# mfkiwl/erlangnetwork-gnsslib-sdr

Measured on AMD Instinct MI355X. Metric: correlations/sec (1 ms coh) + x real-time, 32-SV L1CA @16.368 Msps, higher is better.
Workload: dtype int8 samples x int8 carrier LUT -> int32 accumulators (exact); NCOs: the reference's fp64 running sums, bit for bit; 1 GPU; BASELINE configs[2]: 32-SV GPS L1CA tracking, 5-tap E/P/L correlators (CORRN=2, CORRD=3), 1 ms coherent, 16.368 Msps int8 IQ, per GPU; channels_per_gpu=32, epochs_per_launch=1000, taps=5, loop=open (frequencies held per launch); see closed_loop (--full), if_broadcast=none (1 GPU)

## Files before the change

### erlangnetwork-gnsslib-sdr_amd/csrc/gnsscorr_nco.h

```cpp
#pragma once

#include <math.h>
#include <stdint.h>
#include <string.h>
#include <type_traits>

#if defined(__HIPCC__)
#define GC_HD __host__ __device__ inline
#define GC_HDM __host__ __device__
#define GC_HD_NOINLINE __host__ __device__ __attribute__((noinline))
#else
#define GC_HD static inline
#define GC_HDM
#define GC_HD_NOINLINE static
#endif
#if defined(__clang__)
#define GC_FP_STRICT _Pragma("clang fp contract(off)")
#else
#define GC_FP_STRICT
#endif

#if defined(__HIP_DEVICE_COMPILE__)
#define GC_DDIV(a, b) __ddiv_rn((a), (b))
#else
// ... 567 lines not shown
    } else if (!(reach < gc_u2d((uint64_t)(f.ex0 + GC_NB) << 52))) {
        return false;
    }
    c->exact = gc_cert_exact(x, f.s, reach);
    *pi0 = i0;
    *pilim = ilim;
    return true;
}

struct GcFillLoop {
    GC_HDM bool operator()(int *K, const GcCertCtx &c, int i0, int itop, double lim) const
    {
        int prev = 0;
        for (int i = i0 + 1; i <= GC_NB; i++) {
            K[i] = (i <= itop || i == GC_NB) ? gc_cert_lane(c, i, lim) : GC_CERT_FAR;
            if (K[i] == GC_CERT_FAIL) return false;
            if (i <= itop || i == GC_NB) {
                if (K[i] <= prev && !(K[i] == GC_CERT_FAR && (i != GC_NB || !(lim < 1.0e300)))) return false;
                prev = K[i];
            }
        }
        return true;
    }
};

#if defined(__HIPCC__)
struct GcFillLanes {
    int lane;
    __device__ bool operator()(int *K, const GcCertCtx &c, int i0, int itop, double lim) const
    {
        int Kl = GC_CERT_FAR;
        const bool mine = lane > i0 && lane <= GC_NB && (lane <= itop || lane == GC_NB);
        if (mine) Kl = gc_cert_lane(c, lane, lim);
        const int src = lane == GC_NB ? itop : lane - 1;
        const int below = __shfl(Kl, src < 0 ? 0 : src, 64);
        const bool bad = mine && (Kl == GC_CERT_FAIL || (src > i0 && Kl <= below && !(Kl == GC_CERT_FAR && (lane != GC_NB || !(lim < 1.0e300)))) || Kl <= 0);
        if (__any(bad)) return false;
#pragma unroll
        for (int i = 0; i <= GC_NB; i++) K[i] = __builtin_amdgcn_readlane(Kl, i);
        return true;
    }
};
#endif

template <class Fill>
GC_HD bool gc_cert_stretch(const GcNcoFast &f, double *px, int *pk, int n, double lim, Fill &fill)
{
    GcCertCtx c;
    int i0, ilim;
    if (!gc_cert_setup(f, *px, *pk, n, lim, &c, &i0, &ilim)) return false;
    const int klim = gc_cert_lane(c, GC_NB, lim);
    if (klim == GC_CERT_FAIL) return false;
    int K[GC_NB + 1];
    if (!fill(K, c, i0, ilim, klim == GC_CERT_FAR ? INFINITY : lim)) return false;
    double y = *px;
    int k = 0;
    if (!gc_cert_chain(f, &y, &k, c.n, i0, K, ilim, K[GC_NB])) return false;
    *px = y;
    *pk += k;
    return true;
}

template <class Fill>
GC_HD bool gc_plan_code_walk(const GcNcoFast &f, double c, int len, int nt, Fill &fill, double *cend)
{
    GC_FP_STRICT
    const double ci = f.s, dlen = (double)len;
    if (f.ex0 == GC_NO_TABLE || !(ci > 0.0)) return false;
    int j = 0;
    while (j < nt) {
        if (c >= dlen) c = c - dlen;
        while (j < nt && c < dlen && (c == 0.0 || gc_expo(c) < f.ex0)) {
            c = c + ci;
            j += 1;
        }
        if (j >= nt) break;
        if (c >= dlen) continue;
        if (!(c > 0.0) || !gc_cert_stretch(f, &c, &j, nt, dlen, fill)) return false;
    }
    *cend = c;
    return true;
}

GC_HD bool gc_one_binade_walk(double x, double s, int n, double *xn, double *dout = nullptr, bool *tie_out = nullptr)
{
    GC_FP_STRICT
    const uint64_t ux = gc_d2u(x), us = gc_d2u(s);
    if (tie_out) *tie_out = false;
    const int ex = gc_expo(x), es = gc_expo(s);
    if (ex == 0 || ex == 0x7FF || es == 0 || es == 0x7FF || (ux >> 63) != (us >> 63)) return false;
    const int et = es + 1075 - ex;
    if (et >= 1023 + 51) return false;
    double b = 0.0;
    if (et >= 1023 - 1) {
        const double t = gc_u2d((us & 0x800FFFFFFFFFFFFFull) | ((uint64_t)et << 52));
        b = rint(t);
        if (tie_out) *tie_out = fabs(t - b) == 0.5;
        if (fabs(t - b) == 0.5 && (ux & 1)) return false;
    }
    const double d = ldexp(b, ex - 1075);
    const double y = fma((double)n, d, x);
    const double top = fabs(gc_u2d(ux | 0x000FFFFFFFFFFFFFull));
    if (!(fabs(y) <= top)) return false;
    *xn = y;
    if (dout) *dout = d;
    return true;
}

template <class Fill>
GC_HD bool gc_plan_carrier_walk(const GcNcoFast &f, double x, int n, Fill &fill, double *xn)
{
    GC_FP_STRICT
    if (f.ex0 == GC_NO_TABLE) return false;
    if (gc_expo(x) >= f.ex0 + GC_NB) return gc_one_binade_walk(x, f.s, n, xn);
    int k = 0;
    while (k < n && (x == 0.0 || gc_expo(x) < f.ex0)) {
        x = x + f.s;
        k += 1;
    }
    if (k < n && !gc_cert_stretch(f, &x, &k, n, INFINITY, fill)) return false;
    if (k != n) return false;
    *xn = x;
    return true;
}

GC_HD bool gc_plan_code_walk(const GcNcoFast &f, double c, int len, int nt, int *, double *cend)
{
    GcFillLoop fill;
    return gc_plan_code_walk(f, c, len, nt, fill, cend);
}
GC_HD bool gc_plan_carrier_walk(const GcNcoFast &f, double x, int n, int *, double *xn)
{
    GcFillLoop fill;
    return gc_plan_carrier_walk(f, x, n, fill, xn);
}

struct GcCodePlan {
    GcNcoFast f;
    double dlen;
    double limtop;
    double smaxci;
    int    itop;
    int    it;
    bool   exact;
    bool   ok;
};

GC_HD void gc_code_plan_shape(GcCodePlan &P, double ci, int len, int smax)
{
    GC_FP_STRICT
    P.dlen = (double)len;
    P.smaxci = (double)smax * ci;
    P.limtop = gc_u2d(gc_d2u(P.dlen) - 1);
    P.itop = gc_expo(P.limtop) - P.f.ex0;
    P.ok = P.f.ex0 != GC_NO_TABLE && ci > 0.0 && P.itop >= 1 && P.itop < GC_NB &&
           P.dlen + ci < gc_u2d((uint64_t)(P.f.ex0 + P.itop + 1) << 52) && !((P.f.tie >> P.itop) & 1);
    P.exact = P.ok && gc_cert_exact(P.limtop, ci, P.dlen);
    P.it = -1;
#pragma unroll
    for (int i = 0; i < GC_NB; i++)
        if (((P.f.tie >> i) & 1) && i <= P.itop) P.it = i;
}

GC_HD void gc_code_plan_init(GcCodePlan &P, double ci, int len, int smax, bool with_inv = true)
{
    GC_FP_STRICT
    gc_fast_init(P.f, ci, with_inv);
    gc_code_plan_shape(P, ci, len, smax);
    if (P.ok && !with_inv) {
#pragma unroll
        for (int i = 0; i < GC_NB; i++)
            if (i == P.itop && P.f.d[i] != 0.0) P.f.inv[i] = 1.0 / fabs(P.f.d[i]);
    }
}

template <int ITOP, class Emit>
GC_HD void gc_code_climb_lean(const GcNcoFast &f, const int *K, int i0, int it, double ci, double *py, int jbase, Emit &emit)
{
    GC_FP_STRICT
    double y = *py;
#pragma unroll
    for (int i = 0; i <= ITOP; i++) {
        if (i == 0 && i0 != 0) continue;
// ... 208 lines not shown
GC_HD bool gc_carrier_period(const GcCarPlan &P, double remcarr, int n, Fill &fill, double *remcarr_out)
{
    GcNoEmit ne;
    return gc_carrier_period(P, remcarr, n, fill, remcarr_out, ne);
}

enum { GC_TIER_PERIOD = 3, GC_TIER_STRETCH = 4, GC_TIER_WALKER = 5 };

template <class Fill, class Emit, bool STRETCH = std::is_same<Emit, GcNoEmit>::value>
GC_HD double gc_code_period_any(const GcCodePlan &P, double remcode, int nt, Fill &fill, Emit &emit, int *tier)
{
    GC_FP_STRICT
    double r;
    *tier = GC_TIER_PERIOD;
    if (gc_code_period(P, remcode, nt, fill, &r, emit)) return r;
    emit.reset();
    const int len = (int)P.dlen;
    const double c0 = gc_code_start_fast(remcode, P.smaxci, len);
    *tier = GC_TIER_STRETCH;
    if (!(STRETCH && gc_plan_code_walk(P.f, c0, len, nt, fill, &r))) {
        *tier = GC_TIER_WALKER;
        r = gc_fast_code_walk(P.f, c0, len, nt, emit);
    }
    return r - P.smaxci;
}

template <class Fill, class Emit, bool STRETCH = std::is_same<Emit, GcNoEmit>::value>
GC_HD double gc_carrier_period_any(const GcCarPlan &P, double remcarr, int n, Fill &fill, Emit &emit, int *tier)
{
    GC_FP_STRICT
    double r;
    *tier = GC_TIER_PERIOD;
    if (gc_carrier_period(P, remcarr, n, fill, &r, emit)) return r;
    emit.reset();
    const double phis = gc_div_y(remcarr * GC_NCO_CDIV, GC_NCO_DPI, P.ydpi);
    *tier = GC_TIER_STRETCH;
    if (!(STRETCH && gc_plan_carrier_walk(P.f, phis, n, fill, &r))) {
        *tier = GC_TIER_WALKER;
        r = gc_fast_carrier_walk(P.f, phis, n, emit);
    }
    return gc_fast_prem(P.fprem, r);
}

GC_HD void gc_spec_start(double remcode0, double remcarr0, double ci, double spc, double ps, double dlen, int e,
                         double *remcode_e, double *remcarr_e, int *n_e)
{
    GC_FP_STRICT
    const double de = (double)e;
    const double N0 = e == 0 ? 0.0 : floor((de * dlen - remcode0) / spc);
    const double N1 = floor(((de + 1.0) * dlen - remcode0) / spc);
    const double dn = N1 - N0;
    *n_e = (dn > 0.0 && dn < 2147483648.0) ? (int)dn : 0;
    const double p = N0 * ci, pe = fma(N0, ci, -p);
    *remcode_e = (remcode0 + (p - de * dlen)) + pe;
    const double w = ps * GC_NCO_DPI * (1.0 / GC_NCO_CDIV);
    const double q = N0 * w, qe = fma(N0, w, -q);
    double phi = remcarr0 + q;
    if (phi > GC_NCO_DPI && phi < 1.0e300) {
        const double M = ceil(phi / GC_NCO_DPI) - 1.0;
        phi = fma(-M, GC_NCO_DPI, phi);
    }
    *remcarr_e = phi + qe;
}

#define GC_CLAIM_ROW   24
#define GC_CLAIM_LIT   5
#define GC_CLAIM_TAIL  15
#define GC_CLAIM_TAIL2 32
#define GC_CLAIM_CLIT  8
#define GC_CLAIM_CSEG  13
#define GC_CLAIM_PREM  12

GC_HD constexpr int gc_tail_class(int smax) { return smax + 1 > 8 ? (smax + 1 > GC_CLAIM_TAIL ? 2 : 1) : 0; }
GC_HD constexpr int gc_tail_max(int cls) { return cls == 0 ? 8 : (cls == 1 ? GC_CLAIM_TAIL : GC_CLAIM_TAIL2); }

struct GcCodeClaims {
    int tag;
    int i0, q, nl, jsum;
    int dm[13];
    int n, pad;
    double lo, hi;
};

struct GcCarClaims {
    int tag;
    int nl, i0, nseg, kprem;
    int dm[GC_CLAIM_CSEG];
    int pad[2];
    double lo, hi;
};

#if defined(__HIP_DEVICE_COMPILE__)
#define GC_PIN_V(x) asm volatile("" : "+v"(x))
#else
#define GC_PIN_V(x) do { } while (0)
#endif
#if defined(__HIP_DEVICE_COMPILE__)
#define GC_UNIFORM_INT(x) __builtin_amdgcn_readfirstlane(x)
#else
#define GC_UNIFORM_INT(x) (x)
#endif
template <int N>
GC_HD double gc_pick(const double (&a)[N], int idx)
{
#if defined(__HIP_DEVICE_COMPILE__)
    static_assert(N <= 48, "gc_pick: at most 48 values");
    if constexpr (N <= 16) {
        typedef double gc_vecn __attribute__((ext_vector_type(N)));
        gc_vecn v;
#pragma unroll
        for (int i = 0; i < N; i++) v[i] = a[i];
        return v[idx < N ? idx : N - 1];
    } else {
        typedef double gc_vec16 __attribute__((ext_vector_type(16)));
        constexpr int NC = (N + 15) / 16;
        double r = 0.0;
#pragma unroll
        for (int c = 0; c < NC; c++) {
            gc_vec16 v;
#pragma unroll
            for (int i = 0; i < 16; i++) v[i] = a[c * 16 + i < N ? c * 16 + i : N - 1];
            const double rc = v[idx & 15];
            r = (idx >> 4) == c ? rc : r;
        }
        return r;
    }
#else
    return a[idx];
#endif
}

template <int ITOP>
struct GcCodeStepC {
    double d[ITOP + 1], pre[ITOP + 1];
    double ci, dlen, b0, smaxci;
    int    ex_top;
    int    it;
};

template <int ITOP>
GC_HD void gc_code_stepc_init(GcCodeStepC<ITOP> &C, const GcCodePlan &P)
{
    C.ci = P.f.s;
    C.dlen = P.dlen;
    C.b0 = gc_u2d((uint64_t)P.f.ex0 << 52);
    C.smaxci = P.smaxci;
    C.ex_top = P.f.ex0 + ITOP;
    C.it = P.it;
#pragma unroll
    for (int i = 0; i <= ITOP; i++) {
        C.d[i] = P.f.d[i];
        C.pre[i] = i == P.it ? P.f.s : 0.0;
        GC_PIN_V(C.d[i]);
        GC_PIN_V(C.pre[i]);
    }
    GC_PIN_V(C.ci);
    GC_PIN_V(C.dlen);
    GC_PIN_V(C.b0);
    GC_PIN_V(C.smaxci);
}

template <int ITOP, int TMAX, bool DISCOVER, bool PERLANE = DISCOVER>
GC_HD bool gc_code_claims_step(const GcCodePlan &P, const GcCodeStepC<ITOP> &C, double remcode, int nt, GcCodeClaims &cl,
                               double *remcode_out, const double *dmd = nullptr)
{
    GC_FP_STRICT
// ... 291 lines not shown
        prev = p;
        p = p - GC_NCO_DPI;
    }
    *held = (p < 1.0e300) & (kprem >= 0) & (kprem <= GC_CLAIM_PREM) & ((kprem == 0) | (prev > GC_NCO_DPI)) & !(p > GC_NCO_DPI);
    return p;
}

template <int ITOP, int TMAX>
GC_HD double gc_code_value_step(const GcCodeStepC<ITOP> &C, double remcode, int nt, int q, int nl, int i0, int jsum,
                                const double *dmd)
{
    GC_FP_STRICT
    const double ci = C.ci, dlen = C.dlen;
    const int it = GC_UNIFORM_INT(C.it);
    const double cs = remcode - C.smaxci;
    const double c0 = cs < 0.0 ? cs + dlen : cs;
    double y = fma((double)q + 1.0, C.d[ITOP], c0);
    y = y - dlen;
    y = gc_add_n<GC_CLAIM_LIT>(y, ci, nl);
    if (i0 == 0) {
        if (it == 0) y = y + ci;
        y = fma(dmd[0], C.d[0], y);
        y = y + ci;
        GC_PIN_V(y);
    }
    if (it <= 0) {
#pragma unroll
        for (int i = 1; i <= ITOP; i++) {
            y = fma(dmd[i], C.d[i], y);
            y = y + ci;
        }
    } else {
#pragma unroll
        for (int i = 1; i <= ITOP; i++) {
            y = y + C.pre[i];
            y = fma(dmd[i], C.d[i], y);
            y = y + ci;
        }
    }
    y = y - dlen;
    y = gc_add_n<TMAX>(y, ci, nt - jsum);
    return y - C.smaxci;
}

GC_HD double gc_carrier_value_step(const GcCarPlan &P, const GcCarStepC &C, double remcarr, int p0, int plast, int kprem,
                                   const double *dmd)
{
    GC_FP_STRICT
    static_assert(GC_CLAIM_CWIN <= 32, "gc_carrier_value_step: one bit per window position");
    const int ptie = GC_UNIFORM_INT(C.ptie);
    double x = gc_div_y(remcarr * GC_NCO_CDIV, GC_NCO_DPI, P.ydpi);
    const unsigned act = ((2u << (plast - p0)) - 1u) << p0;
    constexpr int PH = GC_CLAIM_CWIN / 2;
    if (ptie < 0) {
        if (p0 < PH) {
#pragma unroll
            for (int p = 0; p < PH; p++)
                if ((act >> p) & 1u) { x = fma(dmd[p], C.d[p], x); x = x + C.s; GC_PIN_V(x); }
        }
#pragma unroll
        for (int p = PH; p < GC_CLAIM_CWIN; p++)
            if ((act >> p) & 1u) { x = fma(dmd[p], C.d[p], x); x = x + C.s; GC_PIN_V(x); }
    } else {
#pragma unroll
        for (int p = 0; p < GC_CLAIM_CWIN; p++)
            if ((act >> p) & 1u) { x = x + C.pre[p]; x = fma(dmd[p], C.d[p], x); x = x + C.s; GC_PIN_V(x); }
    }
    return gc_prem_value(x, kprem);
}

GC_HD bool gc_carrier_value_step_one(const GcCarPlan &P, const GcCarStepC &C, double remcarr, int n, int kprem,
                                     double *remcarr_out)
{
    GC_FP_STRICT
    if (C.ex0 == GC_NO_TABLE || n < 1) return false;
    double x = gc_div_y(remcarr * GC_NCO_CDIV, GC_NCO_DPI, P.ydpi);
    if (!gc_one_binade_walk(x, C.s, n, &x)) return false;
    bool held;
    const double p = gc_prem_checked(x, kprem, &held);
    if (!held) return false;
    *remcarr_out = p;
    return true;
}
```

### erlangnetwork-gnsslib-sdr_amd/csrc/gnsscorr_plan.hip

```cpp
#include <cstdlib>
#include <cstddef>
#include <hip/hip_runtime.h>

#include "gnsscorr_internal.h"

namespace {


#define GC_SPEC_WC  9.313225746154785e-10
#define GC_SPEC_WK  9.313225746154785e-10

struct SpecChan {
    GcCodePlan PC;
    GcCarPlan PK;
    GcCarStepC CK;
    double ci, spc, ps, dlen;
    int clen, smax;
    int tmax;
    bool ok;
};

__device__ __forceinline__ void spec_chan_init(SpecChan &C, const GcChan &c, const GcTrkState &s, bool with_prem)
{
    C.ci = __dmul_rn(c.ti, s.codefreq);
// ... 71 lines not shown
    shk[tid] = pk;
    __syncthreads();
    for (int st = GC_SPEC_CHUNK / 2; st > 0; st >>= 1) {
        if (tid < st) { shc[tid] += shc[tid + st]; shk[tid] += shk[tid + st]; }
        __syncthreads();
    }
    const double basec = shc[0], basek = shk[0];
    __syncthreads();
    shc[tid] = e < T ? devc[(size_t)ch * T + e] : 0.0;
    shk[tid] = e < T ? devk[(size_t)ch * T + e] : 0.0;
    __syncthreads();
    for (int st = 1; st < GC_SPEC_CHUNK; st <<= 1) {
        const double ac = tid >= st ? shc[tid - st] : 0.0, ak = tid >= st ? shk[tid - st] : 0.0;
        __syncthreads();
        shc[tid] += ac;
        shk[tid] += ak;
        __syncthreads();
    }
    if (eb >= nepoch) return;
    const double sumc = basec + (tid ? shc[tid - 1] : 0.0), sumk = basek + (tid ? shk[tid - 1] : 0.0);
    const GcTrkState s = state_in[ch];
    SpecChan C;
    spec_chan_init(C, chan[ch], s, false);
    GcCodeClaims cc;
    GcCarClaims ck;
    cc.tag = 0;
    ck.tag = 0;
    cc.n = cc.pad = 0;
    cc.lo = cc.hi = ck.lo = ck.hi = 0.0;
    if (C.ok) {
        double r0, g0;
        int nhat;
        gc_spec_start(s.remcode, s.remcarr, C.ci, C.spc, C.ps, C.dlen, e, &r0, &g0, &nhat);
        const double rt = r0 + sumc, gt = g0 + sumk;
        int ncode = 0;
        bool bracketed = false;
#pragma unroll 1
        for (int att = 0; att < 2 && !bracketed; att++) {
            const double w = att == 0 ? GC_SPEC_WC : GC_SPEC_WC * 0.00390625;
            const double lo = rt - w, hi = rt + w;
            const int nlo = gc_period_nsamp(C.dlen, lo, C.spc), nhi = gc_period_nsamp(C.dlen, hi, C.spc);
            if (!(nlo == nhi && nlo > 0 && nlo <= (1 << 24))) continue;
            double dummy;
            const bool side = (lo - C.PC.smaxci < 0.0) == (hi - C.PC.smaxci < 0.0);
            const bool oklo = gc_code_claims<true>(C.PC, lo, nlo + 2 * C.smax, cc, &dummy);
            const bool okhi = oklo && gc_code_claims<false>(C.PC, hi, nlo + 2 * C.smax, cc, &dummy);
            const bool tailfits = nlo + 2 * C.smax - cc.jsum <= C.tmax;
            if (side && oklo && okhi && tailfits) {
                bracketed = true;
                ncode = nlo;
                cc.tag = 1;
                cc.n = nlo;
                cc.lo = lo;
                cc.hi = hi;
            }
        }
        if (!bracketed) {
            ncode = gc_period_nsamp(C.dlen, rt, C.spc);
            cc.tag = 0;
            if (ncode > 0 && ncode <= (1 << 24)) {
                double dummy;
                cc.tag = (gc_code_claims<true>(C.PC, rt, ncode + 2 * C.smax, cc, &dummy) && ncode + 2 * C.smax - cc.jsum <= C.tmax) ? 3 : 0;
            }
            cc.n = ncode;
            cc.lo = cc.hi = rt;
        }
        const int nk = ncode;
        if (nk > 0 && nk <= (1 << 24)) {
            bool kbr = false;
            int tag = 0;
#pragma unroll 1
            for (int att = 0; att < 2 && !kbr; att++) {
                const double w = fmax(GC_SPEC_WK, fabs(gt) * 1.4551915228366852e-11) * (att == 0 ? 1.0 : 0.00390625);
                const double klo = gt - w, khi = gt + w;
                double dummy;
                bool ok = gc_carrier_claims_step<true>(C.PK, C.CK, klo, nk, ck, &dummy);
                tag = ck.tag;
                ok = ok && gc_carrier_claims_step<false, true>(C.PK, C.CK, khi, nk, ck, &dummy);
                if (ok) {
                    kbr = true;
                    ck.tag = tag;
                    ck.lo = klo;
                    ck.hi = khi;
                }
            }
            if (!kbr) {
                double dummy;
                const bool ok = gc_carrier_claims_step<true>(C.PK, C.CK, gt, nk, ck, &dummy);
                ck.tag = ok ? (ck.tag == 2 ? 2 : 3) : 0;
                ck.lo = ck.hi = gt;
            }
            ck.nl = nk;
        }
    }
    const size_t row = (size_t)ch * nepoch + eb;
    int4 *rc = reinterpret_cast<int4 *>(claims_code) + row * (GC_CLAIM_ROW / 4);
    int4 *rk = reinterpret_cast<int4 *>(claims_car) + row * (GC_CLAIM_ROW / 4);
    const int4 *pc4 = reinterpret_cast<const int4 *>(&cc), *pk4 = reinterpret_cast<const int4 *>(&ck);
#pragma unroll
    for (int q = 0; q < GC_CLAIM_ROW / 4; q++) {
        rc[q] = pc4[q];
        rk[q] = pk4[q];
    }
}

__device__ unsigned long long gc_plan_stats[8];

__host__ __device__ inline int plan2_class(double ti, double codefreq, int clen, int smax)
{
    const double ci = ti * codefreq;
    if (!(ci > 0.0) || !gc_fast_has_table(ci)) return -1;
    const int itop = gc_expo(gc_u2d(gc_d2u((double)clen) - 1)) - (gc_expo(ci) + 2);
    if (itop < 7 || itop > 12) return -1;
    if (smax + 1 > GC_CLAIM_TAIL2) return -1;
    return (itop - 7) * 3 + gc_tail_class(smax);
}

#define GC_PLAN_MAXE 4096
__device__ __attribute__((noinline)) void trk_plan_body(const GcChan *__restrict__ chan,
                                                        const GcTrkState *__restrict__ state_in,
                                                        GcTrkState *__restrict__ state_out,
                                                        GcTrkPlan *__restrict__ plan, int nch, int nepoch)
{
    __shared__ int nsh[GC_PLAN_MAXE];
    __shared__ int prog;
    const int ch = blockIdx.x, lane = threadIdx.x & 63, wave = threadIdx.x >> 6;
    if (ch >= nch) return;
    __builtin_amdgcn_s_setprio(3);
    const bool split = nepoch <= GC_PLAN_MAXE;
    if (threadIdx.x == 0) prog = 0;
    __syncthreads();
    if (!split && wave == 1) return;
    const GcChan c = chan[ch];
    GcTrkState s = state_in[ch];
    const double ci = __dmul_rn(c.ti, s.codefreq);
    const double spc = __ddiv_rn(s.codefreq, c.f_sf);
    const double ps = gc_carrier_ps(s.carrfreq, c.ti);
    const double dlen = (double)c.clen;
    const bool code_ok = ci > 0.0 && ci < dlen;
    GcTrkPlan *out = plan + (size_t)ch * nepoch;
    GcNoEmit ne;
    GcFillLanes fill{lane};
    const bool do_code = wave == 0, do_car = wave == 1 || !split;
    GcCodePlan PC;
    GcCarPlan PK;
    if (do_code) gc_code_plan_init(PC, ci, c.clen, c.smax);
    if (do_car) gc_car_plan_init(PK, ps);
    const double yspc = gc_period_yspc(spc);
    unsigned tally[6] = {0, 0, 0, 0, 0, 0};
    for (int e = 0; e < nepoch; e++) {
        int n;
        if (do_code) {
            n = gc_period_nsamp(dlen, s.remcode, spc, yspc);
            if (lane == 0) {
                out[e].buffloc = s.buffloc;
                out[e].coff = s.remcode;
                out[e].carrfreq = s.carrfreq;
                out[e].codefreq = s.codefreq;
                out[e].n = n;
                out[e].pad = 0;
            }
            if (split) {
                if (lane == 0) nsh[e] = n;
                __threadfence_block();
                if (lane == 0) __hip_atomic_store(&prog, e + 1, __ATOMIC_RELEASE, __HIP_MEMORY_SCOPE_WORKGROUP);
            }
        } else {
            while (__hip_atomic_load(&prog, __ATOMIC_ACQUIRE, __HIP_MEMORY_SCOPE_WORKGROUP) <= e) __builtin_amdgcn_s_sleep(1);
            n = nsh[e];
        }
        const bool walk = n > 0 && n <= (1 << 24);
        if (do_car) {
            if (lane == 0) out[e].phi0 = s.remcarr;
            if (walk) {
                int tier;
                s.remcarr = gc_carrier_period_any(PK, s.remcarr, n, fill, ne, &tier);
                if (tier == GC_TIER_PERIOD) tally[4]++;
                else tally[5]++;
            }
        }
        if (do_code) {
            if (walk && code_ok) {
                int tier;
                s.remcode = gc_code_period_any(PC, s.remcode, n + 2 * c.smax, fill, ne, &tier);
                if (tier == GC_TIER_PERIOD) tally[1]++;
                else tally[2]++;
            }
            s.buffloc += (uint64_t)(int64_t)n;
        }
// ... 157 lines not shown
    const int v = __hip_atomic_load(&g_plan4.prog, __ATOMIC_RELAXED, __HIP_MEMORY_SCOPE_WORKGROUP);
    asm volatile("" ::: "memory");
    return v;
}
template <int ITOP, int TMAX>
__device__ __attribute__((noinline)) int plan4_code_other(double ci_, int clen_, int smax_, double remcode_, int n_, int lane, const GcCodeClaims *cl_, double *out)
{
    const GcCodeClaims *clp = plan2_uni(cl_);
    if (plan2_uni(clp->tag) == 1 || plan2_uni(clp->tag) == 3) {
        const double ci = plan2_uni(ci_), remcode = plan2_uni(remcode_);
        const int clen = plan2_uni(clen_), smax = plan2_uni(smax_), n = plan2_uni(n_);
        GcCodePlan PC;
        gc_code_plan_init(PC, ci, clen, smax, false);
        GcCodeStepC<ITOP> SC;
        gc_code_stepc_init(SC, PC);
        GcCodeClaims c2 = *clp;
        c2.tag = 1;
        double rc;
        if (gc_code_claims_step<ITOP, TMAX, false, true>(PC, SC, remcode, n + 2 * smax, c2, &rc)) { *out = rc; return 0; }
    }
    return plan2_code_slow(ci_, clen_, smax_, remcode_, n_, lane, out);
}

__device__ __forceinline__ int plan4_scopy(int x)
{
    int c;
    asm volatile("s_mov_b32 %0, %1" : "=s"(c) : "s"(x));
    return c;
}
__device__ __forceinline__ bool plan4_bcopy(bool x) { return __builtin_amdgcn_readfirstlane(x ? 1 : 0) != 0; }

template <int ITOP, int TMAX>
__device__ __attribute__((noinline)) void plan4_code_wave(double ci_, double spc_, int clen_, int smax_, const Plan4Job *J_, int lane)
{
    const int clen = plan2_uni(clen_), smax = plan2_uni(smax_);
    const double ci = plan2_uni(ci_), spc = plan2_uni(spc_);
    const Plan4Job J = plan4_job(J_);
    const double dlen = (double)clen;
    GcCodePlan PC;
    gc_code_plan_init(PC, ci, clen, smax);
    GcCodeStepC<ITOP> SC;
    gc_code_stepc_init(SC, PC);
    const double yspc = __ddiv_rn(1.0, spc);
    const bool fastdiv = spc > 1e-300 && spc < 1e300 && yspc < 1e300;
    unsigned tally0 = 0, tally1 = 0, tally2 = 0, miss = 0, mism = 0;
    GC_GLOBAL GcTrkPlan *out = (GC_GLOBAL GcTrkPlan *)J.out;
    double remcode = J.s.remcode;
    unsigned long long buffloc = J.s.buffloc;
    GC_PP_DECL;
    GC_PP_T0(ptot_);
    for (int b = 0; b < J.nblk; b++) {
        const int nb = plan4_nb(J, b), e0 = b * GC_P4_BLK;
        const GC_CONST gc_v4i *rows = (const GC_CONST gc_v4i *)J.claims_code + (size_t)e0 * (GC_CLAIM_ROW / 4);
        GcCodeClaims row = plan4_code_row(rows);
        for (int i = 0; i < nb; i++) {
            __builtin_amdgcn_s_waitcnt(0xC07F);
            const double num = __dsub_rn(dlen, remcode);
            double qn = gc_div_y(num, spc, yspc);
            if (__builtin_expect(!fastdiv, 0)) qn = __ddiv_rn(num, spc);
            const int n = plan2_uni((qn > -2147483648.0 && qn < 2147483648.0) ? (int)qn : 0);
            const int tag = row.tag;
            const bool inside = tag == 1 && remcode >= row.lo && remcode <= row.hi && n == row.n;
            double dmd[ITOP + 1];
            const int q = plan4_scopy(row.q), nl = plan4_scopy(row.nl), i0 = plan4_scopy(row.i0);
            const int jsum = plan4_scopy(row.jsum);
#pragma unroll
            for (int k = 0; k <= ITOP; k++) {
                dmd[k] = (double)row.dm[k];
                GC_PIN_V(dmd[k]);
            }
            const bool inside_u = plan4_bcopy(inside);
            const bool claims_u = plan4_bcopy(tag == 1);
            __builtin_amdgcn_sched_barrier(0);
            if (i + 1 < nb) row = plan4_code_row(rows + (i + 1) * (GC_CLAIM_ROW / 4));
            __builtin_amdgcn_sched_barrier(0);
            if (lane == 0) {
                g_plan4.vstart[0][i] = remcode;
                g_plan4.vbuff[i] = buffloc;
                g_plan4.nsh[e0 + i] = n;
                plan4_publish(e0 + i + 1);
            }
            if (n > 0 && n <= (1 << 24)) {
                double rc = remcode;
                if (inside_u && !J.verify) {
                    rc = gc_code_value_step<ITOP, TMAX>(SC, remcode, n + 2 * smax, q, nl, i0, jsum, dmd);
                    tally0++;
                } else {
                    double rs;
                    GC_PP_T0(pslow_);
                    const int how = plan4_code_other<ITOP, TMAX>(ci, clen, smax, remcode, n, lane,
                                                                 reinterpret_cast<const GcCodeClaims *>(J.claims_code) + e0 + i, &rs);
                    GC_PP_ADD(1, pslow_);
                    GC_PP_INC(4);
                    tally0 += how == 0 ? 1 : 0;
                    tally1 += how == 1 ? 1 : 0;
                    tally2 += how == 2 ? 1 : 0;
                    mism += (inside_u && how != 0) ? 1 : 0;
                    miss += (!inside_u && claims_u) ? 1 : 0;
                    rc = rs;
                }
                remcode = rc;
            }
            buffloc += (unsigned long long)(long long)n;
        }
        if (lane < nb) {
            GC_GLOBAL GcTrkPlan *o = out + e0 + lane;
            o->buffloc = g_plan4.vbuff[lane];
            o->coff = g_plan4.vstart[0][lane];
            o->carrfreq = J.s.carrfreq;
            o->codefreq = J.s.codefreq;
            o->n = g_plan4.nsh[e0 + lane];
            o->pad = 0;
        }
    }
    GC_PP_ADD(0, ptot_);
    GC_PP_OUT(0);
    if (lane == 0) {
        GC_GLOBAL GcTrkState *so = (GC_GLOBAL GcTrkState *)J.state_out;
        so->carrfreq = J.s.carrfreq;
        so->codefreq = J.s.codefreq;
        so->remcode = remcode;
        so->buffloc = buffloc;
        if (tally0) atomicAdd(&gc_plan_stats[0], (unsigned long long)tally0);
        if (tally1) atomicAdd(&gc_plan_stats[1], (unsigned long long)tally1);
        if (tally2) atomicAdd(&gc_plan_stats[2], (unsigned long long)tally2);
        if (mism) atomicAdd(&gc_plan_stats[6], (unsigned long long)mism);
        if (miss) atomicAdd(&gc_plan_stats[7], (unsigned long long)miss);
    }
}

__device__ __attribute__((noinline)) int plan4_car_other(double ps_, int nsamp_, double remcarr_, int n_, int lane, const GcCarClaims *cl_, double *out)
{
    const GcCarClaims *clp = plan2_uni(cl_);
    const int tag = plan2_uni(clp->tag);
    if (tag != 0) {
        const double ps = plan2_uni(ps_), remcarr = plan2_uni(remcarr_);
        const int n = plan2_uni(n_), nsamp = plan2_uni(nsamp_);
        GcCarPlan PK;
        gc_car_plan_init(PK, ps, false, false);
        GcCarStepC CK;
        gc_car_stepc_init(CK, PK, nsamp + 16);
        GcCarClaims c2 = *clp;
        c2.tag = tag == 2 ? 2 : 1;
        double rp;
        if (gc_carrier_claims_step<false, true>(PK, CK, remcarr, n, c2, &rp)) { *out = rp; return 0; }
    }
    return plan2_car_slow(remcarr_, n_, lane, out);
}

__device__ __attribute__((noinline)) void plan4_car_cert_wave(double ps_, const Plan4Job *J_, int lane)
{
    const double ps = plan2_uni(ps_);
    const Plan4Job J = plan4_job(J_);
    GcCarPlan PK;
    gc_car_plan_init(PK, ps);
    GcFillLanes fill{lane};
    GcNoEmit ne;
    unsigned tally1 = 0, tally2 = 0;
    GC_GLOBAL GcTrkPlan *out = (GC_GLOBAL GcTrkPlan *)J.out;
    double remcarr = J.s.remcarr;
    int seen = 0;
    for (int b = 0; b < J.nblk; b++) {
        const int nb = plan4_nb(J, b), e0 = b * GC_P4_BLK;
        for (int i = 0; i < nb; i++) {
            while (seen <= e0 + i) {
                seen = plan2_uni(plan4_progress());
                if (seen <= e0 + i) __builtin_amdgcn_s_sleep(1);
            }
            const int n = plan2_uni(g_plan4.nsh[e0 + i]);
            if (lane == 0) g_plan4.vstart[1][i] = remcarr;
            if (n > 0 && n <= (1 << 24)) {
                int tier;
                remcarr = gc_carrier_period_any(PK, remcarr, n, fill, ne, &tier);
                tally1 += tier == GC_TIER_PERIOD ? 1 : 0;
                tally2 += tier == GC_TIER_PERIOD ? 0 : 1;
            }
        }
        if (lane < nb) out[e0 + lane].phi0 = g_plan4.vstart[1][lane];
    }
    if (lane == 0) {
        ((GC_GLOBAL GcTrkState *)J.state_out)->remcarr = remcarr;
        if (tally1) atomicAdd(&gc_plan_stats[4], (unsigned long long)tally1);
        if (tally2) atomicAdd(&gc_plan_stats[5], (unsigned long long)tally2);
    }
}

__device__ __attribute__((noinline)) void plan4_car_wave(double ps_, int nsamp_, const Plan4Job *J_, int lane)
{
    const int nsamp = plan2_uni(nsamp_);
    const double ps = plan2_uni(ps_);
    const Plan4Job J = plan4_job(J_);
    {
        const int nlook = J.nepoch < 16 ? J.nepoch : 16;
        int none = 0;
        for (int e = 0; e < nlook; e++)
            none += ((const GC_CONST int *)J.claims_car)[(size_t)e * GC_CLAIM_ROW] == 0 ? 1 : 0;
        if (none == nlook && nlook >= 8) {
            plan4_car_cert_wave(ps, J_, lane);
            return;
        }
    }
    {
        GcCarPlan full;
        gc_car_plan_init(full, ps);
        if (lane == 0) g_plan4.pkfull = full;
    }
    GcCarPlan PK;
    gc_car_plan_init(PK, ps, false, false);
    GcCarStepC CK;
    gc_car_stepc_init(CK, PK, nsamp + 16);
    const int ilo = plan2_uni(CK.ilo);
    unsigned tally0 = 0, tally1 = 0, tally2 = 0, miss = 0, mism = 0;
    GC_GLOBAL GcTrkPlan *out = (GC_GLOBAL GcTrkPlan *)J.out;
    double remcarr = J.s.remcarr;
    int seen = 0;
    GC_PP_DECL;
    GC_PP_T0(ptot_);
    for (int b = 0; b < J.nblk; b++) {
        const int nb = plan4_nb(J, b), e0 = b * GC_P4_BLK;
        const GC_CONST gc_v4i *rows = (const GC_CONST gc_v4i *)J.claims_car + (size_t)e0 * (GC_CLAIM_ROW / 4);
        GcCarClaims row = plan4_car_row(rows);
        for (int i = 0; i < nb; i++) {
            GC_PP_T0(ptop_);
            if (seen <= e0 + i) {
                GC_PP_T0(pn_);
                while (seen <= e0 + i) {
                    seen = plan2_uni(plan4_progress());
                    if (seen <= e0 + i) __builtin_amdgcn_s_sleep(1);
                }
                GC_PP_ADD(3, pn_);
            }
            const int n = plan2_uni(g_plan4.nsh[e0 + i]);
            __builtin_amdgcn_s_waitcnt(0xC07F);
            const int tag = row.tag;
            const bool inside = tag == 1 && remcarr >= row.lo && remcarr <= row.hi && n == row.nl;
            double dmd[GC_CLAIM_CWIN];
            const int p0 = plan4_scopy(row.i0 - ilo);
            const int plast = plan4_scopy(row.i0 - ilo + row.nseg - 1);
            const int kprem = plan4_scopy(row.kprem);
#pragma unroll
            for (int k = 0; k < GC_CLAIM_CWIN; k++) {
                dmd[k] = (double)row.dm[k];
                GC_PIN_V(dmd[k]);
            }
            const bool inside_u = plan4_bcopy(inside);
            const int tag_u = plan4_scopy(tag);
            __builtin_amdgcn_sched_barrier(0);
            if (i + 1 < nb) row = plan4_car_row(rows + (i + 1) * (GC_CLAIM_ROW / 4));
            __builtin_amdgcn_sched_barrier(0);
            if (lane == 0) g_plan4.vstart[1][i] = remcarr;
            GC_PP_ADD(5, ptop_);
            GC_PP_T0(pstep_);
            if (n > 0 && n <= (1 << 24)) {
                double rp = remcarr;
                bool done = false;
                if (inside_u && !J.verify) {
                    rp = gc_carrier_value_step(PK, CK, remcarr, p0, plast, kprem, dmd);
                    done = true;
                } else if (tag_u == 2) {
                    double r2 = remcarr;
                    done = gc_carrier_value_step_one(PK, CK, remcarr, n, kprem, &r2);
                    rp = done ? r2 : rp;
                }
                if (done) {
                    tally0++;
                } else {
                    double rs;
                    GC_PP_T0(pslow_);
                    const int how = plan4_car_other(ps, nsamp, remcarr, n, lane, reinterpret_cast<const GcCarClaims *>(J.claims_car) + e0 + i, &rs);
                    GC_PP_ADD(1, pslow_);
                    GC_PP_INC(4);
                    tally0 += how == 0 ? 1 : 0;
                    tally1 += how == 1 ? 1 : 0;
                    tally2 += how == 2 ? 1 : 0;
                    mism += (inside_u && how != 0) ? 1 : 0;
                    miss += (!inside_u && tag_u == 1) ? 1 : 0;
                    rp = rs;
                }
                remcarr = rp;
            }
            GC_PP_ADD(6, pstep_);
        }
        if (lane < nb) out[e0 + lane].phi0 = g_plan4.vstart[1][lane];
    }
    GC_PP_ADD(0, ptot_);
    GC_PP_OUT(1);
    if (lane == 0) {
        ((GC_GLOBAL GcTrkState *)J.state_out)->remcarr = remcarr;
        if (tally0) atomicAdd(&gc_plan_stats[3], (unsigned long long)tally0);
        if (tally1) atomicAdd(&gc_plan_stats[4], (unsigned long long)tally1);
        if (tally2) atomicAdd(&gc_plan_stats[5], (unsigned long long)tally2);
        if (mism) atomicAdd(&gc_plan_stats[6], (unsigned long long)mism);
        if (miss) atomicAdd(&gc_plan_stats[7], (unsigned long long)miss);
    }
}

template <int ITOP>
__device__ __forceinline__ void plan4_code_dispatch(int tcls, double ci, double spc, int clen, int smax, const Plan4Job *J, int lane)
{
    if (tcls == 0) plan4_code_wave<ITOP, gc_tail_max(0)>(ci, spc, clen, smax, J, lane);
    else if (tcls == 1) plan4_code_wave<ITOP, gc_tail_max(1)>(ci, spc, clen, smax, J, lane);
    else plan4_code_wave<ITOP, gc_tail_max(2)>(ci, spc, clen, smax, J, lane);
}

__global__ __launch_bounds__(128) void trk_plan4_kernel(const GcChan *__restrict__ chan, const GcTrkState *__restrict__ state_in,
                                                        GcTrkState *__restrict__ state_out, GcTrkPlan *__restrict__ plan,
                                                        int nch, int nepoch, const int *__restrict__ claims_code,
                                                        const int *__restrict__ claims_car, int verify)
{
    const int ch = blockIdx.x, tid = threadIdx.x, lane = tid & 63, wave = tid >> 6;
    if (ch >= nch) return;
    const GcChan c = chan[ch];
    const GcTrkState s = state_in[ch];
    const double ci = __dmul_rn(c.ti, s.codefreq), spc = __ddiv_rn(s.codefreq, c.f_sf), ps = gc_carrier_ps(s.carrfreq, c.ti);
    const int cls = plan2_class(c.ti, s.codefreq, c.clen, c.smax);
    if (cls < 0 || !(ci > 0.0 && ci < (double)c.clen)) {
        trk_plan_body(chan, state_in, state_out, plan, nch, nepoch);
        return;
    }
    const int itop = cls / 3 + 7, tcls = cls % 3;
    constexpr int RW4 = GC_CLAIM_ROW / 4;
    Plan4Job J;
    J.claims_code = reinterpret_cast<const int4 *>(claims_code) + (size_t)ch * nepoch * RW4;
    J.claims_car = reinterpret_cast<const int4 *>(claims_car) + (size_t)ch * nepoch * RW4;
    J.out = plan + (size_t)ch * nepoch;
    J.state_out = state_out + ch;
    J.s = s;
    J.nepoch = nepoch;
    J.nblk = (nepoch + GC_P4_BLK - 1) / GC_P4_BLK;
    J.verify = verify;
    if (tid == 0) g_plan4.prog = 0;
    __syncthreads();
    __builtin_amdgcn_s_setprio(3);
    if (wave == 0) {
        gc_with_itop(itop, [&](auto IT) { plan4_code_dispatch<decltype(IT)::value>(tcls, ci, spc, c.clen, c.smax, &J, lane); return true; });
    } else {
        plan4_car_wave(ps, c.nsamp, &J, lane);
    }
}


}


#ifdef GC_PLAN_PROF
extern "C" int gnsscorr_debug_plan_prof(unsigned long long *dst)
{
    if (hipMemcpyFromSymbol(dst, HIP_SYMBOL(gc_plan_prof), sizeof(unsigned long long) * 64 * 16) != hipSuccess) return -1;
    return 0;
}
#endif

extern "C" int gnsscorr_debug_plan_stats(unsigned long long *dst, int reset)
{
    if (hipMemcpyFromSymbol(dst, HIP_SYMBOL(gc_plan_stats), sizeof(unsigned long long) * 8) != hipSuccess) return -1;
    if (reset) {
        unsigned long long z[8] = {0, 0, 0, 0, 0, 0, 0, 0};
        if (hipMemcpyToSymbol(HIP_SYMBOL(gc_plan_stats), z, sizeof(z)) != hipSuccess) return -1;
    }
    return 0;
}

static bool trk_nospec()
{
    static const bool nospec = getenv("GNSSCORR_TRK_NOSPEC") != nullptr;
    return nospec;
}

size_t gc_trk_spec_ints(size_t units) { return units * (2 * GC_CLAIM_ROW + 8); }

int gc_launch_trk_spec(hipStream_t st, const GcChan *chan, const GcTrkState *state_in, int nch, int nepoch, int *claims,
                       int e_off)
{
    if (!claims || trk_nospec() || nepoch > GC_PLAN_MAXE || e_off < 0 || e_off > nepoch) return 0;
    const size_t units = (size_t)nch * nepoch;
    const int T = e_off + nepoch;
    double *devc = reinterpret_cast<double *>(claims + 2 * units * GC_CLAIM_ROW), *devk = devc + 2 * units;
    hipLaunchKernelGGL(trk_specdev_kernel, dim3((nch * T + 63) / 64), dim3(64), 0, st, chan, state_in, devc, devk, nch, T);
    GC_HIP(hipGetLastError());
    const int nchunk = (nepoch + GC_SPEC_CHUNK - 1) / GC_SPEC_CHUNK;
    hipLaunchKernelGGL(trk_spec_kernel, dim3(nch * nchunk), dim3(GC_SPEC_CHUNK), 0, st, chan, state_in, devc, devk, claims,
                       claims + units * GC_CLAIM_ROW, nch, nepoch, e_off);
    GC_HIP(hipGetLastError());
    return 0;
}

int gc_launch_trk_plan(hipStream_t st, const GcChan *chan, const GcTrkState *state_in, GcTrkState *state_out,
                       GcTrkPlan *plan, int nch, int nepoch, int *claims)
{
    static const int verify = getenv("GNSSCORR_PLAN_VERIFY") ? atoi(getenv("GNSSCORR_PLAN_VERIFY")) : 0;
    const bool batch = claims && !trk_nospec() && nepoch <= GC_PLAN_MAXE;
    if (batch)
        hipLaunchKernelGGL(trk_plan4_kernel, dim3(nch), dim3(128), 0, st, chan, state_in, state_out, plan, nch, nepoch,
                           claims, claims + (size_t)nch * nepoch * GC_CLAIM_ROW, verify);
    else
        hipLaunchKernelGGL(trk_plan_kernel, dim3(nch), dim3(128), 0, st, chan, state_in, state_out, plan, nch, nepoch);
    GC_HIP(hipGetLastError());
    return 0;
}
```

Before: 265.4 million correlations/s.

## Run carrier planner speculatively on claimed sample counts, validate per block, memoize binade step

The carrier wave no longer waits on the code wave's published sample count for each epoch when a claim row exists. It uses the claimed count, checks it against the real counts once per block, and redoes the block via the slow path if any differ. It also memoizes the one-binade step increment keyed on the exponent bits, and adds a fast kprem==0 path. This lets carrier and code planning overlap instead of lock-stepping, at the cost of a full block recompute on any mismatch and extra complexity in verify flag handling.

```diff
diff --git a/erlangnetwork-gnsslib-sdr_amd/csrc/gnsscorr_nco.h b/erlangnetwork-gnsslib-sdr_amd/csrc/gnsscorr_nco.h
--- a/erlangnetwork-gnsslib-sdr_amd/csrc/gnsscorr_nco.h
+++ b/erlangnetwork-gnsslib-sdr_amd/csrc/gnsscorr_nco.h
@@ -673,11 +673,12 @@
     return true;
 }
 
-GC_HD bool gc_one_binade_walk(double x, double s, int n, double *xn, double *dout = nullptr, bool *tie_out = nullptr)
+GC_HD bool gc_one_binade_step(double x, double s, double *d, bool *tie)
 {
     GC_FP_STRICT
     const uint64_t ux = gc_d2u(x), us = gc_d2u(s);
-    if (tie_out) *tie_out = false;
+    *tie = false;
+    *d = 0.0;
     const int ex = gc_expo(x), es = gc_expo(s);
     if (ex == 0 || ex == 0x7FF || es == 0 || es == 0x7FF || (ux >> 63) != (us >> 63)) return false;
     const int et = es + 1075 - ex;
@@ -686,10 +687,22 @@
     if (et >= 1023 - 1) {
         const double t = gc_u2d((us & 0x800FFFFFFFFFFFFFull) | ((uint64_t)et << 52));
         b = rint(t);
-        if (tie_out) *tie_out = fabs(t - b) == 0.5;
-        if (fabs(t - b) == 0.5 && (ux & 1)) return false;
-    }
-    const double d = ldexp(b, ex - 1075);
+        *tie = fabs(t - b) == 0.5;
+    }
+    *d = ldexp(b, ex - 1075);
+    return true;
+}
+
+GC_HD bool gc_one_binade_walk(double x, double s, int n, double *xn, double *dout = nullptr, bool *tie_out = nullptr)
+{
+    GC_FP_STRICT
+    const uint64_t ux = gc_d2u(x);
+    double d;
+    bool tie;
+    const bool has = gc_one_binade_step(x, s, &d, &tie);
+    if (tie_out) *tie_out = tie;
+    if (!has) return false;
+    if (tie && (ux & 1)) return false;
     const double y = fma((double)n, d, x);
     const double top = fabs(gc_u2d(ux | 0x000FFFFFFFFFFFFFull));
     if (!(fabs(y) <= top)) return false;
@@ -1521,3 +1534,50 @@
     *remcarr_out = p;
     return true;
 }
+
+struct GcOneBinadeMemo {
+    uint32_t key;
+    int has, tie;
+    double d;
+};
+GC_HD void gc_one_binade_memo_init(GcOneBinadeMemo &M) { M.key = 0; M.has = M.tie = 0; M.d = 0.0; }
+
+GC_HD bool gc_one_binade_walk_memo(GcOneBinadeMemo &M, double x, double s, int n, double *xn)
+{
+    GC_FP_STRICT
+    const uint64_t ux = gc_d2u(x);
+    const uint32_t key = (uint32_t)GC_UNIFORM_INT((int)(gc_hi32(x) & 0xFFF00000u));
+    if (key != M.key || key == 0) {
+        bool tie;
+        M.has = gc_one_binade_step(x, s, &M.d, &tie) ? 1 : 0;
+        M.tie = tie ? 1 : 0;
+        M.key = key;
+    }
+    if (!M.has) return false;
+    if (M.tie && (ux & 1)) return false;
+    const double y = fma((double)n, M.d, x);
+    const double top = fabs(gc_u2d(ux | 0x000FFFFFFFFFFFFFull));
+    if (!(fabs(y) <= top)) return false;
+    *xn = y;
+    return true;
+}
+
+GC_HD bool gc_carrier_value_step_one_memo(const GcCarPlan &P, const GcCarStepC &C, GcOneBinadeMemo &M, double remcarr, int n,
+                                          int kprem, double *remcarr_out)
+{
+    GC_FP_STRICT
+    if (C.ex0 == GC_NO_TABLE || n < 1) return false;
+    double x = gc_div_y(remcarr * GC_NCO_CDIV, GC_NCO_DPI, P.ydpi);
+    if (!gc_one_binade_walk_memo(M, x, C.s, n, &x)) return false;
+    double p;
+    bool held;
+    if (kprem == 0) {
+        p = x * GC_NCO_DPI * (1.0 / GC_NCO_CDIV);
+        held = (p < 1.0e300) & !(p > GC_NCO_DPI);
+    } else {
+        p = gc_prem_checked(x, kprem, &held);
+    }
+    if (!held) return false;
+    *remcarr_out = p;
+    return true;
+}
diff --git a/erlangnetwork-gnsslib-sdr_amd/csrc/gnsscorr_plan.hip b/erlangnetwork-gnsslib-sdr_amd/csrc/gnsscorr_plan.hip
--- a/erlangnetwork-gnsslib-sdr_amd/csrc/gnsscorr_plan.hip
+++ b/erlangnetwork-gnsslib-sdr_amd/csrc/gnsscorr_plan.hip
@@ -523,7 +523,7 @@
             }
             if (n > 0 && n <= (1 << 24)) {
                 double rc = remcode;
-                if (inside_u && !J.verify) {
+                if (inside_u && !(J.verify & 1)) {
                     rc = gc_code_value_step<ITOP, TMAX>(SC, remcode, n + 2 * smax, q, nl, i0, jsum, dmd);
                     tally0++;
                 } else {
@@ -626,6 +626,31 @@
     }
 }
 
+__device__ __attribute__((noinline)) double plan4_car_redo(double ps, int nsamp, double remcarr_, const Plan4Job *J_, int e0_, int nb_, int lane,
+                                                            unsigned *t0, unsigned *t1, unsigned *t2)
+{
+    const Plan4Job J = plan4_job(J_);
+    const int e0 = plan2_uni(e0_), nb = plan2_uni(nb_);
+    double remcarr = plan2_uni(remcarr_);
+    unsigned a0 = 0, a1 = 0, a2 = 0;
+    for (int i = 0; i < nb; i++) {
+        const int n = plan2_uni(g_plan4.nsh[e0 + i]);
+        if (lane == 0) g_plan4.vstart[1][i] = remcarr;
+        if (n > 0 && n <= (1 << 24)) {
+            double rs;
+            const int how = plan4_car_other(ps, nsamp, remcarr, n, lane, reinterpret_cast<const GcCarClaims *>(J.claims_car) + e0 + i, &rs);
+            a0 += how == 0 ? 1 : 0;
+            a1 += how == 1 ? 1 : 0;
+            a2 += how == 2 ? 1 : 0;
+            remcarr = plan2_uni(rs);
+        }
+    }
+    *t0 = a0;
+    *t1 = a1;
+    *t2 = a2;
+    return remcarr;
+}
+
 __device__ __attribute__((noinline)) void plan4_car_wave(double ps_, int nsamp_, const Plan4Job *J_, int lane)
 {
     const int nsamp = plan2_uni(nsamp_);
@@ -650,6 +675,8 @@
     gc_car_plan_init(PK, ps, false, false);
     GcCarStepC CK;
     gc_car_stepc_init(CK, PK, nsamp + 16);
+    GcOneBinadeMemo memo;
+    gc_one_binade_memo_init(memo);
     const int ilo = plan2_uni(CK.ilo);
     unsigned tally0 = 0, tally1 = 0, tally2 = 0, miss = 0, mism = 0;
     GC_GLOBAL GcTrkPlan *out = (GC_GLOBAL GcTrkPlan *)J.out;
@@ -661,20 +688,24 @@
         const int nb = plan4_nb(J, b), e0 = b * GC_P4_BLK;
         const GC_CONST gc_v4i *rows = (const GC_CONST gc_v4i *)J.claims_car + (size_t)e0 * (GC_CLAIM_ROW / 4);
         GcCarClaims row = plan4_car_row(rows);
+        const double remcarr_b = remcarr;
+        const unsigned b0 = tally0, b1 = tally1, b2 = tally2, bmiss = miss, bmism = mism;
         for (int i = 0; i < nb; i++) {
             GC_PP_T0(ptop_);
-            if (seen <= e0 + i) {
+            __builtin_amdgcn_s_waitcnt(0xC07F);
+            const int tag = row.tag;
+            int n = plan4_scopy(row.nl);
+            if (tag == 0) {
                 GC_PP_T0(pn_);
                 while (seen <= e0 + i) {
                     seen = plan2_uni(plan4_progress());
                     if (seen <= e0 + i) __builtin_amdgcn_s_sleep(1);
                 }
                 GC_PP_ADD(3, pn_);
-            }
-            const int n = plan2_uni(g_plan4.nsh[e0 + i]);
-            __builtin_amdgcn_s_waitcnt(0xC07F);
-            const int tag = row.tag;
-            const bool inside = tag == 1 && remcarr >= row.lo && remcarr <= row.hi && n == row.nl;
+                n = plan2_uni(g_plan4.nsh[e0 + i]);
+                __builtin_amdgcn_s_waitcnt(0xC07F);
+            }
+            const bool inside = tag == 1 && remcarr >= row.lo && remcarr <= row.hi;
             double dmd[GC_CLAIM_CWIN];
             const int p0 = plan4_scopy(row.i0 - ilo);
             const int plast = plan4_scopy(row.i0 - ilo + row.nseg - 1);
@@ -695,12 +726,12 @@
             if (n > 0 && n <= (1 << 24)) {
                 double rp = remcarr;
                 bool done = false;
-                if (inside_u && !J.verify) {
+                if (inside_u && !(J.verify & 1)) {
                     rp = gc_carrier_value_step(PK, CK, remcarr, p0, plast, kprem, dmd);
                     done = true;
                 } else if (tag_u == 2) {
                     double r2 = remcarr;
-                    done = gc_carrier_value_step_one(PK, CK, remcarr, n, kprem, &r2);
+                    done = gc_carrier_value_step_one_memo(PK, CK, memo, remcarr, n, kprem, &r2);
                     rp = done ? r2 : rp;
                 }
                 if (done) {
@@ -722,6 +753,28 @@
             }
             GC_PP_ADD(6, pstep_);
         }
+        {
+            GC_PP_T0(pn_);
+            while (seen < e0 + nb) {
+                seen = plan2_uni(plan4_progress());
+                if (seen < e0 + nb) __builtin_amdgcn_s_sleep(1);
+            }
+            GC_PP_ADD(3, pn_);
+            bool differs = false;
+            if (lane < nb) {
+                const int *r = reinterpret_cast<const int *>(J.claims_car) + (size_t)(e0 + lane) * GC_CLAIM_ROW;
+                differs = r[0] != 0 && r[1] != g_plan4.nsh[e0 + lane];
+            }
+            if (__ballot(differs) != 0ull || (J.verify & 4)) {
+                unsigned r0, r1, r2;
+                remcarr = plan4_car_redo(ps, nsamp, remcarr_b, J_, e0, nb, lane, &r0, &r1, &r2);
+                tally0 = b0 + r0;
+                tally1 = b1 + r1;
+                tally2 = b2 + r2;
+                miss = bmiss;
+                mism = bmism;
+            }
+        }
         if (lane < nb) out[e0 + lane].phi0 = g_plan4.vstart[1][lane];
     }
     GC_PP_ADD(0, ptot_);
```

Result: slower. 246.4 million correlations/s (-7.2%).

## Precompute proven single-binade carrier step during speculation to skip runtime walk

Applied to the files above, without the earlier changes.

During carrier speculation, when a tag-2 (single-binade) claim's bracket endpoints can be shown to share an exponent with a fixed rounding increment, the planner stores that increment in the claim row under a new tag. The planning wave then computes the carrier phase with a single fma and prem instead of running the checked binade walk. The aim is to cut fp64 work in the serial carrier plan loop. The cost is extra proof work in the speculative kernel, more branch paths, and new debug counters.

```diff
diff --git a/erlangnetwork-gnsslib-sdr_amd/csrc/gnsscorr_nco.h b/erlangnetwork-gnsslib-sdr_amd/csrc/gnsscorr_nco.h
--- a/erlangnetwork-gnsslib-sdr_amd/csrc/gnsscorr_nco.h
+++ b/erlangnetwork-gnsslib-sdr_amd/csrc/gnsscorr_nco.h
@@ -1064,6 +1064,7 @@
     double lo, hi;
 };
 
+#define GC_CAR_TAG_ONE_PROVEN 4
 struct GcCarClaims {
     int tag;
     int nl, i0, nseg, kprem;
@@ -1521,3 +1522,49 @@
     *remcarr_out = p;
     return true;
 }
+
+GC_HD bool gc_one_binade_bracket(const GcCarPlan &P, double s, double klo, double khi, int n, int kprem, double *dout)
+{
+    GC_FP_STRICT
+    if (!(klo <= khi) || n < 1) return false;
+    const double xlo = gc_div_y(klo * GC_NCO_CDIV, GC_NCO_DPI, P.ydpi);
+    const double xhi = gc_div_y(khi * GC_NCO_CDIV, GC_NCO_DPI, P.ydpi);
+    const uint64_t ul = gc_d2u(xlo), uh = gc_d2u(xhi), us = gc_d2u(s);
+    const int ex = gc_expo(xlo), es = gc_expo(s);
+    if (ex == 0 || ex == 0x7FF || es == 0 || es == 0x7FF) return false;
+    if (gc_expo(xhi) != ex || (ul >> 63) != (us >> 63) || (uh >> 63) != (us >> 63)) return false;
+    const int et = es + 1075 - ex;
+    if (et >= 1023 + 51) return false;
+    double b = 0.0;
+    if (et >= 1023 - 1) {
+        const double t = gc_u2d((us & 0x800FFFFFFFFFFFFFull) | ((uint64_t)et << 52));
+        b = rint(t);
+        if (fabs(t - b) == 0.5) return false;
+    }
+    const double d = ldexp(b, ex - 1075);
+    const double top = fabs(gc_u2d(ul | 0x000FFFFFFFFFFFFFull));
+    const double yl = fma((double)n, d, xlo), yh = fma((double)n, d, xhi);
+    if (!(fabs(yl) <= top) || !(fabs(yh) <= top)) return false;
+    bool hl, hh;
+    gc_prem_checked(yl, kprem, &hl);
+    gc_prem_checked(yh, kprem, &hh);
+    if (!hl || !hh) return false;
+    *dout = d;
+    return true;
+}
+
+GC_HD double gc_carrier_value_step_one_bracketed(const GcCarPlan &P, double remcarr, int n, double d, int kprem)
+{
+    GC_FP_STRICT
+    double x = gc_div_y(remcarr * GC_NCO_CDIV, GC_NCO_DPI, P.ydpi);
+    x = fma((double)n, d, x);
+    return gc_prem_value(x, kprem);
+}
+
+GC_HD void gc_car_claims_set_d(GcCarClaims &cl, double d)
+{
+    const uint64_t u = gc_d2u(d);
+    cl.dm[0] = (int)(uint32_t)u;
+    cl.dm[1] = (int)(uint32_t)(u >> 32);
+}
+GC_HD double gc_car_claims_d(int dm0, int dm1) { return gc_u2d(((uint64_t)(uint32_t)dm1 << 32) | (uint32_t)dm0); }
diff --git a/erlangnetwork-gnsslib-sdr_amd/csrc/gnsscorr_plan.hip b/erlangnetwork-gnsslib-sdr_amd/csrc/gnsscorr_plan.hip
--- a/erlangnetwork-gnsslib-sdr_amd/csrc/gnsscorr_plan.hip
+++ b/erlangnetwork-gnsslib-sdr_amd/csrc/gnsscorr_plan.hip
@@ -177,6 +177,11 @@
                     ck.tag = tag;
                     ck.lo = klo;
                     ck.hi = khi;
+                    double d1;
+                    if (tag == 2 && gc_one_binade_bracket(C.PK, C.ps, klo, khi, nk, ck.kprem, &d1)) {
+                        ck.tag = GC_CAR_TAG_ONE_PROVEN;
+                        gc_car_claims_set_d(ck, d1);
+                    }
                 }
             }
             if (!kbr) {
@@ -200,6 +205,7 @@
 }
 
 __device__ unsigned long long gc_plan_stats[8];
+__device__ unsigned long long gc_plan_stats_one[2];
 
 __host__ __device__ inline int plan2_class(double ti, double codefreq, int clen, int smax)
 {
@@ -582,7 +588,7 @@
         GcCarStepC CK;
         gc_car_stepc_init(CK, PK, nsamp + 16);
         GcCarClaims c2 = *clp;
-        c2.tag = tag == 2 ? 2 : 1;
+        c2.tag = (tag == 2 || tag == GC_CAR_TAG_ONE_PROVEN) ? 2 : 1;
         double rp;
         if (gc_carrier_claims_step<false, true>(PK, CK, remcarr, n, c2, &rp)) { *out = rp; return 0; }
     }
@@ -651,6 +657,7 @@
     GcCarStepC CK;
     gc_car_stepc_init(CK, PK, nsamp + 16);
     const int ilo = plan2_uni(CK.ilo);
+    unsigned one0 = 0, one1 = 0;
     unsigned tally0 = 0, tally1 = 0, tally2 = 0, miss = 0, mism = 0;
     GC_GLOBAL GcTrkPlan *out = (GC_GLOBAL GcTrkPlan *)J.out;
     double remcarr = J.s.remcarr;
@@ -674,7 +681,7 @@
             const int n = plan2_uni(g_plan4.nsh[e0 + i]);
             __builtin_amdgcn_s_waitcnt(0xC07F);
             const int tag = row.tag;
-            const bool inside = tag == 1 && remcarr >= row.lo && remcarr <= row.hi && n == row.nl;
+            const bool inb = (tag == 1 || tag == GC_CAR_TAG_ONE_PROVEN) && remcarr >= row.lo && remcarr <= row.hi && n == row.nl;
             double dmd[GC_CLAIM_CWIN];
             const int p0 = plan4_scopy(row.i0 - ilo);
             const int plast = plan4_scopy(row.i0 - ilo + row.nseg - 1);
@@ -684,8 +691,9 @@
                 dmd[k] = (double)row.dm[k];
                 GC_PIN_V(dmd[k]);
             }
-            const bool inside_u = plan4_bcopy(inside);
+            const bool inb_u = plan4_bcopy(inb);
             const int tag_u = plan4_scopy(tag);
+            const bool inside_u = inb_u && tag_u == 1, inside1_u = inb_u && tag_u == GC_CAR_TAG_ONE_PROVEN;
             __builtin_amdgcn_sched_barrier(0);
             if (i + 1 < nb) row = plan4_car_row(rows + (i + 1) * (GC_CLAIM_ROW / 4));
             __builtin_amdgcn_sched_barrier(0);
@@ -698,10 +706,17 @@
                 if (inside_u && !J.verify) {
                     rp = gc_carrier_value_step(PK, CK, remcarr, p0, plast, kprem, dmd);
                     done = true;
-                } else if (tag_u == 2) {
+                } else if (inside1_u && !J.verify) {
+                    const double d1 = gc_car_claims_d((int)dmd[0], (int)dmd[1]);
+                    rp = gc_carrier_value_step_one_bracketed(PK, remcarr, n, d1, kprem);
+                    done = true;
+                    one0++;
+                } else if (tag_u == 2 || tag_u == GC_CAR_TAG_ONE_PROVEN) {
                     double r2 = remcarr;
                     done = gc_carrier_value_step_one(PK, CK, remcarr, n, kprem, &r2);
                     rp = done ? r2 : rp;
+                    one1++;
+                    mism += (inside1_u && !done) ? 1 : 0;
                 }
                 if (done) {
                     tally0++;
@@ -733,6 +748,8 @@
         if (tally2) atomicAdd(&gc_plan_stats[5], (unsigned long long)tally2);
         if (mism) atomicAdd(&gc_plan_stats[6], (unsigned long long)mism);
         if (miss) atomicAdd(&gc_plan_stats[7], (unsigned long long)miss);
+        if (one0) atomicAdd(&gc_plan_stats_one[0], (unsigned long long)one0);
+        if (one1) atomicAdd(&gc_plan_stats_one[1], (unsigned long long)one1);
     }
 }
 
@@ -802,6 +819,16 @@
     return 0;
 }
 
+extern "C" int gnsscorr_debug_plan_stats_one(unsigned long long dst[2], int reset)
+{
+    if (hipMemcpyFromSymbol(dst, HIP_SYMBOL(gc_plan_stats_one), sizeof(unsigned long long) * 2) != hipSuccess) return -1;
+    if (reset) {
+        unsigned long long z[2] = {0, 0};
+        if (hipMemcpyToSymbol(HIP_SYMBOL(gc_plan_stats_one), z, sizeof(z)) != hipSuccess) return -1;
+    }
+    return 0;
+}
+
 static bool trk_nospec()
 {
     static const bool nospec = getenv("GNSSCORR_TRK_NOSPEC") != nullptr;
```

Measured after the change: 267.1 million correlations/s before, 268.4 million correlations/s after, median of 2. No clear change (+0.5%).
